# adityamwagh/SuperSLAM

Hardware: AMD Instinct MI355X
Metric: stereo pairs/sec (SPx2+LG) at 1376x376 (higher is better)
Workload: dtype f16; 1 GPU; configs[1]: SuperPoint x2 + select + gather + 1x LightGlue on 1376x376 stereo pairs; a step = 8 x 64 = 512 pairs per GPU resident in HBM (8 library calls of 64 pairs, different images per call), max_keypoints 600, seeded synthetic weights; pairs_per_call=64, max_keypoints=600, matches_last_call=1412, parallelism=replicated weights, pairs sharded over 1 rank(s), no data-path collective

## Files before the change

superslam_amd/csrc/api.hip:

```cpp
#include <algorithm>
#include <atomic>
#include <cmath>
#include <cstdarg>
#include <cstdlib>
#include <cstring>
#include <fstream>
#include <map>
#include <memory>
#include <mutex>
#include <string>
#include <vector>

#include "../../include/sship.h"
#include "../../include/superslam_hip/place_recognizer.hpp"
#include "kernels.h"

namespace sship {

static thread_local std::string g_err;
static void (*g_log_cb)(int, const char*) = nullptr;
static int g_profiling = 0;

void set_error(const std::string& msg) {
  g_err = msg;
// ... 492 lines not shown
  t.cand = cand.as<unsigned long long>(); t.cand_count = cnt.as<int>(); t.cap = cap; t.max_kp = max_kp;
  t.score_w = score_w;
  t.scale_x = static_cast<float>(input_w) / score_w;
  t.scale_y = static_cast<float>(input_h) / score_h;
  t.desc_h = desc_h; t.desc_w = desc_w; t.kp_xys = kp_xys; t.cell_h = cell_h; t.cell_w = cell_w; t.n_out = n_dev;
  t.n_cand_out = n_cand_dev;
  launch_topk(t, 1, s);
  SSHIP_HIP_CHECK(hipGetLastError());
  SSHIP_HIP_CHECK(hipStreamSynchronize(s));
  return SSHIP_OK;
}

struct sship_sp {
  sship_sp_config cfg{};
  hipStream_t stream = nullptr;
  float* w1a = nullptr;
  float* b1a = nullptr;
  _Float16* w1a_frag = nullptr;
  _Float16* w1a_fragb = nullptr;
  ConvW c1b, c2a, c2b, c3a, c3b, c4a, c4b, cPa, cPb, cDa, cDb;
  ConvW cDb32;
  sship_pool* pool = nullptr;
  int wsB = 0, wsH = 0, wsW = 0;
  DevBuf img, a1a, a1b, a2a, a2b, a3a, a3b, a4a, a4b, aPa, aDa, draw, logits, cand, cand_count;
  const void* cand_zero_ptr = nullptr; int cand_zero_n = 0;
  hipStream_t cand_zero_stream = nullptr;
  DevBuf kp, cell_h, cell_w, n_dev, desc_stage, gray_in;
  PinBuf h_kp, h_n, h_img;
  int cap = 0;
  float thr_f = 0.f;
  bool img_valid = false;
  struct Ring {
    int depth = 0, h = 0, w = 0, ch = 0;
    size_t img_bytes = 0;
    std::vector<void*> host, dev;
    std::vector<hipEvent_t> uploaded;
    hipStream_t copy_stream = nullptr;
    struct Pending { bool active = false; int slots[2] = {-1, -1}; int rc_pool = 0; hipEvent_t done = nullptr; void* h_kp = nullptr; void* h_n = nullptr; };
    std::vector<Pending> pending;
  } ring;
};

static void ring_free(sship_sp* sp);
static void sp_shapes(int H, int W, int& H2, int& W2, int& H4, int& W4, int& Hc, int& Wc) {
  H2 = H / 2; W2 = W / 2; H4 = H2 / 2; W4 = W2 / 2; Hc = H4 / 2; Wc = W4 / 2;
}

static int sp_ensure(sship_sp* sp, int B, int H, int W) {
  if (B <= sp->wsB && H == sp->wsH && W == sp->wsW) return SSHIP_OK;
  int H2, W2, H4, W4, Hc, Wc;
  sp_shapes(H, W, H2, W2, H4, W4, Hc, Wc);
  if (Hc < 1 || Wc < 1) return fail(SSHIP_ERR_INVALID, "image too small for SuperPoint (needs >= 8x8)");
  const size_t px1 = (size_t)B * H * W, px2 = (size_t)B * H2 * W2, px4 = (size_t)B * H4 * W4, pxc = (size_t)B * Hc * Wc;
  const int mk = sp->cfg.max_keypoints;
  SSHIP_HIP_CHECK(sp->img.ensure(px1));
  SSHIP_HIP_CHECK(sp->gray_in.ensure(px1 * 3));
  SSHIP_HIP_CHECK(sp->a1a.ensure(px1 * 64 * 2));
  SSHIP_HIP_CHECK(sp->a1b.ensure(px2 * 64 * 2));
  SSHIP_HIP_CHECK(sp->a2a.ensure(px2 * 64 * 2));
  SSHIP_HIP_CHECK(sp->a2b.ensure(px4 * 64 * 2));
  SSHIP_HIP_CHECK(sp->a3a.ensure(px4 * 128 * 2));
  SSHIP_HIP_CHECK(sp->a3b.ensure(pxc * 128 * 2));
  SSHIP_HIP_CHECK(sp->a4a.ensure(pxc * 128 * 2));
  SSHIP_HIP_CHECK(sp->a4b.ensure(pxc * 128 * 2));
  SSHIP_HIP_CHECK(sp->aPa.ensure(pxc * 256 * 2));
  SSHIP_HIP_CHECK(sp->aDa.ensure(pxc * 256 * 2));
  SSHIP_HIP_CHECK(sp->draw.ensure(pxc * 256 * 2));
  SSHIP_HIP_CHECK(sp->logits.ensure(pxc * kLogitStride * 4));
  sp->cap = Hc * 8 * Wc * 8;
  SSHIP_HIP_CHECK(sp->cand.ensure((size_t)B * sp->cap * 8));
  SSHIP_HIP_CHECK(sp->cand_count.ensure((size_t)B * 4));
  SSHIP_HIP_CHECK(sp->kp.ensure((size_t)B * mk * 3 * 4));
  SSHIP_HIP_CHECK(sp->cell_h.ensure((size_t)B * mk * 4));
  SSHIP_HIP_CHECK(sp->cell_w.ensure((size_t)B * mk * 4));
  SSHIP_HIP_CHECK(sp->n_dev.ensure((size_t)B * 4));
  SSHIP_HIP_CHECK(sp->h_kp.ensure((size_t)B * mk * 3 * 4));
  SSHIP_HIP_CHECK(sp->h_n.ensure((size_t)B * 4));
  SSHIP_HIP_CHECK(sp->h_img.ensure(px1 * 3));
  sp->wsB = B; sp->wsH = H; sp->wsW = W;
  return SSHIP_OK;
}

static int conv_mode() {
  static const int v = [] {
    const char* e = dev_env("SUPERSLAM_HIP_CONV");
    return (SSHIP_DEV_SWITCHES && e && std::string(e) == "strip") ? 2 : 1;
  }();
  return v;
}
static hipError_t conv3(const ConvW& w, const _Float16* in, _Float16* out, int B, int H, int W, bool pool, hipStream_t s) {
#if SSHIP_DEV_SWITCHES
  static const bool wino = [] { const char* e = dev_env("SUPERSLAM_HIP_CONV64"); return e && std::string(e) == "wino"; }();
  if (wino && w.w_wino && sp_conv3x3_wino_fits(H, W, w.cin, w.cout)) return sp_conv3x3_wino(w.w_wino, w.bias, in, out, B, H, W, pool, s);
  return conv_mode() == 1 ? sp_conv3x3_pp(w, in, out, B, H, W, pool, s) : sp_conv3x3_strip(w, in, out, B, H, W, pool, s);
#else
  return sp_conv3x3_pp(w, in, out, B, H, W, pool, s);
#endif
}
static bool conv2_fused(int B, int H2, int W2) {
#if SSHIP_DEV_SWITCHES
  static const std::string mode = [] { const char* e = dev_env("SUPERSLAM_HIP_CONV2"); return std::string(e ? e : ""); }();
  static const bool other = [] { const char* e = dev_env("SUPERSLAM_HIP_CONV64"); return e != nullptr; }();
  if (mode == "split" || other || conv_mode() != 1) return false;
#endif
  return sp_conv2ab_fused_fits(B, H2, W2, true);
}
static hipError_t conv3a_layer(const ConvW& w, const _Float16* in, _Float16* out, int B, int H, int W, hipStream_t s) {
#if SSHIP_DEV_SWITCHES
  static const bool roll = [] { const char* e = dev_env("SUPERSLAM_HIP_CONV3A"); return e && std::string(e) == "roll"; }();
  if (roll && conv_mode() == 1 && w.cin == 64 && w.cout == 128 && w.ct == 64 && sp_conv3a_roll_fits(B, H, W)) return sp_conv3a_roll(w, in, out, B, H, W, s);
#endif
  return conv3(w, in, out, B, H, W, false, s);
}
static hipError_t conv1ab(sship_sp* sp, const uint8_t* img, _Float16* out, int B, int H, int W, hipStream_t s);
static bool desc_dense_mode() {
  static const bool v = [] { const char* e = dev_env("SUPERSLAM_HIP_DESC"); return e && std::string(e) == "dense"; }();
  return v;
}
static hipError_t desc_head(sship_sp* sp, int img0, int Hc, int Wc, const int* cell_h, const int* cell_w, const int* n_dev, int B,
                            _Float16* out, size_t out_img_stride, hipStream_t s) {
  const int mk = sp->cfg.max_keypoints;
  if (desc_dense_mode()) {
    launch_desc_head_gather(sp->cDb32, sp->aDa.as<_Float16>() + (size_t)img0 * Hc * Wc * 256, Hc, Wc, cell_h, cell_w, n_dev, mk, B, out,
                            out_img_stride, s);
    return hipGetLastError();
  }
  return launch_desc_head_sparse(sp->cDa, sp->cDb32, sp->a4b.as<_Float16>() + (size_t)img0 * Hc * Wc * 128, Hc, Wc, cell_h, cell_w, n_dev,
                                 mk, B, out, out_img_stride, s);
}

static int sp_network(sship_sp* sp, const uint8_t* imgs, int B, int H, int W, hipStream_t s, bool dense_desc) {
  int H2, W2, H4, W4, Hc, Wc;
  sp_shapes(H, W, H2, W2, H4, W4, Hc, Wc);
  SSHIP_HIP_CHECK(conv1ab(sp, imgs, sp->a1b.as<_Float16>(), B, H, W, s));
  g_timer.mark_fine("sp_gpu_infer:encoder/conv1a+conv1b+pool", s);
  if (conv2_fused(B, H2, W2)) {
    SSHIP_HIP_CHECK(sp_conv2ab_fused(sp->c2a, sp->c2b, sp->a1b.as<_Float16>(), sp->a2b.as<_Float16>(), B, H2, W2, s));
    g_timer.mark_fine("sp_gpu_infer:encoder/conv2a+conv2b+pool", s);
  } else {
    SSHIP_HIP_CHECK(conv3(sp->c2a, sp->a1b.as<_Float16>(), sp->a2a.as<_Float16>(), B, H2, W2, false, s));
    g_timer.mark_fine("sp_gpu_infer:encoder/conv2a", s);
    SSHIP_HIP_CHECK(conv3(sp->c2b, sp->a2a.as<_Float16>(), sp->a2b.as<_Float16>(), B, H2, W2, true, s));
    g_timer.mark_fine("sp_gpu_infer:encoder/conv2b+pool", s);
  }
  SSHIP_HIP_CHECK(conv3a_layer(sp->c3a, sp->a2b.as<_Float16>(), sp->a3a.as<_Float16>(), B, H4, W4, s));
  g_timer.mark_fine("sp_gpu_infer:encoder/conv3a", s);
  SSHIP_HIP_CHECK(conv3(sp->c3b, sp->a3a.as<_Float16>(), sp->a3b.as<_Float16>(), B, H4, W4, true, s));
  g_timer.mark_fine("sp_gpu_infer:encoder/conv3b+pool", s);
  SSHIP_HIP_CHECK(conv3(sp->c4a, sp->a3b.as<_Float16>(), sp->a4a.as<_Float16>(), B, Hc, Wc, false, s));
  g_timer.mark_fine("sp_gpu_infer:encoder/conv4a", s);
  SSHIP_HIP_CHECK(conv3(sp->c4b, sp->a4a.as<_Float16>(), sp->a4b.as<_Float16>(), B, Hc, Wc, false, s));
  g_timer.mark(g_profiling >= 2 ? "sp_gpu_infer:encoder/conv4b" : "sp_gpu_infer:encoder", s);
  SSHIP_HIP_CHECK(conv3(sp->cPa, sp->a4b.as<_Float16>(), sp->aPa.as<_Float16>(), B, Hc, Wc, false, s));
  g_timer.mark_fine("sp_gpu_infer:heads/convPa", s);
  SSHIP_HIP_CHECK(sp_conv1x1_f32(sp->cPb, sp->aPa.as<_Float16>(), sp->logits.as<float>(), kLogitStride, B, Hc, Wc, s));
  if (dense_desc || desc_dense_mode()) SSHIP_HIP_CHECK(conv3(sp->cDa, sp->a4b.as<_Float16>(), sp->aDa.as<_Float16>(), B, Hc, Wc, false, s));
  if (dense_desc) SSHIP_HIP_CHECK(sp_conv1x1_f16(sp->cDb, sp->aDa.as<_Float16>(), sp->draw.as<_Float16>(), B, Hc, Wc, s));
  g_timer.mark(g_profiling >= 2 ? "sp_gpu_infer:heads/convPb" : "sp_gpu_infer:heads", s);
  return SSHIP_OK;
}

static int sp_select(sship_sp* sp, int B, int H, int W, float* scores_out, float* kp_out, int* n_out, hipStream_t s) {
  int H2, W2, H4, W4, Hc, Wc;
  sp_shapes(H, W, H2, W2, H4, W4, Hc, Wc);
  if (sp->cand_zero_ptr != sp->cand_count.p || sp->cand_zero_n < B || sp->cand_zero_stream != s)
    SSHIP_HIP_CHECK(hipMemsetAsync(sp->cand_count.p, 0, (size_t)B * 4, s));
  sp->cand_zero_ptr = sp->cand_count.p; sp->cand_zero_n = 0; sp->cand_zero_stream = s;
  NmsArgs a{};
  a.logits = sp->logits.as<float>(); a.ls = kLogitStride; a.B = B; a.H = Hc * 8; a.W = Wc * 8;
  a.radius = sp->cfg.nms_radius; a.thr_f = sp->thr_f; a.border = sp->cfg.remove_borders;
  a.cand = sp->cand.as<unsigned long long>(); a.cand_count = sp->cand_count.as<int>(); a.cap = sp->cap;
  a.scores_out = scores_out;
  launch_nms_tile(0, a, s);
  g_timer.mark_fine("sp_extract_stereo:select/nms_tile", s);
  TopkArgs t{};
  t.cand = a.cand; t.cand_count = a.cand_count; t.cap = sp->cap; t.max_kp = sp->cfg.max_keypoints;
  t.score_w = Wc * 8;
  t.scale_x = static_cast<float>(W) / (Wc * 8);
  t.scale_y = static_cast<float>(H) / (Hc * 8);
  t.desc_h = Hc; t.desc_w = Wc; t.kp_xys = kp_out; t.cell_h = sp->cell_h.as<int>(); t.cell_w = sp->cell_w.as<int>();
  t.n_out = n_out; t.n_cand_out = nullptr; t.reset_count = a.cand_count;
  launch_topk(t, B, s);
  SSHIP_HIP_CHECK(hipGetLastError());
  sp->cand_zero_n = B;
  g_timer.mark(g_profiling >= 2 ? "sp_extract_stereo:select/topk" : "sp_extract_stereo:select", s);
  return SSHIP_OK;
}

static hipError_t conv1ab(sship_sp* sp, const uint8_t* img, _Float16* out, int B, int H, int W, hipStream_t s) {
#if SSHIP_DEV_SWITCHES
  if (conv_mode() == 2) return sp_conv1ab_fused(sp->c1b, sp->w1a_frag, sp->b1a, img, out, B, H, W, s);
#endif
  return sp_conv1ab_pp(sp->c1b, sp->w1a_fragb, sp->b1a, img, out, B, H, W, s);
}

extern "C" int sship_sp_create(const sship_sp_config* cfg, sship_sp** out) {
  bind_thread();
  if (!cfg || !out || !cfg->weights_path) return fail(SSHIP_ERR_INVALID, "sp_create: null argument");
  if (cfg->max_keypoints <= 0 || cfg->max_keypoints > kMaxKp) return fail(SSHIP_ERR_INVALID, "sp_create: max_keypoints must be in [1, 4096]");
  if (cfg->nms_radius < 0 || cfg->nms_radius > 8) return fail(SSHIP_ERR_INVALID, "sp_create: nms_radius must be in [0, 8]");
  if (int rc = require_device()) return rc;
  StateDict sd; std::string err;
  if (!load_safetensors(cfg->weights_path, sd, err)) return fail(SSHIP_ERR_IO, err);
  std::unique_ptr<sship_sp, void (*)(sship_sp*)> sp(new sship_sp(), sship_sp_destroy);
// ... 69 lines not shown
  if (int rc = sship_pool_create(sp->cfg.pool_slots, sp->cfg.max_keypoints, SSHIP_DESC_DIM, &sp->pool)) return rc;
  *out = sp.release();
  return SSHIP_OK;
}
extern "C" void sship_sp_destroy(sship_sp* sp) {
  bind_thread();
  if (!sp) return;
  (void)hipDeviceSynchronize();
  for (ConvW* c : {&sp->c1b, &sp->c2a, &sp->c2b, &sp->c3a, &sp->c3b, &sp->c4a, &sp->c4b, &sp->cPa, &sp->cPb, &sp->cDa, &sp->cDb, &sp->cDb32})
    free_conv(*c);
  if (sp->w1a) (void)hipFree(sp->w1a);
  if (sp->b1a) (void)hipFree(sp->b1a);
  if (sp->w1a_frag) (void)hipFree(sp->w1a_frag);
  if (sp->w1a_fragb) (void)hipFree(sp->w1a_fragb);
  ring_free(sp);
  if (sp->pool) sship_pool_destroy(sp->pool);
  sp->pool = nullptr;
  if (sp->stream) (void)hipStreamDestroy(sp->stream);
  delete sp;
}
extern "C" int sship_sp_debug_activation(sship_sp* sp, int layer, void* out_host, unsigned long long bytes) {
  bind_thread();
  if (!sp || !out_host) return fail(SSHIP_ERR_INVALID, "sp_debug_activation: null argument");
  DevBuf* bufs[8] = {nullptr, &sp->a1b, &sp->a2a, &sp->a2b, &sp->a3a, &sp->a3b, &sp->a4a, &sp->a4b};
  if (layer < 1 || layer > 7 || !bufs[layer]->p || bytes > bufs[layer]->bytes) return fail(SSHIP_ERR_INVALID, "sp_debug_activation: bad layer / size");
  SSHIP_HIP_CHECK(hipDeviceSynchronize());
  SSHIP_HIP_CHECK(hipMemcpy(out_host, bufs[layer]->p, bytes, hipMemcpyDeviceToHost));
  return SSHIP_OK;
}
extern "C" sship_pool* sship_sp_pool(sship_sp* sp) {
  bind_thread(); return sp ? sp->pool : nullptr; }
extern "C" int sship_sp_max_keypoints(const sship_sp* sp) { return sp ? sp->cfg.max_keypoints : 0; }

extern "C" int sship_sp_extract_batch_device(sship_sp* sp, const uint8_t* imgs, int batch, int h, int w, void* desc_out,
                                             float* kp_out, int* n_out, void* stream) {
  bind_thread();
  if (!sp || !imgs || !desc_out || !kp_out || !n_out || batch <= 0) return fail(SSHIP_ERR_INVALID, "sp_extract_batch_device: bad arguments");
  hipStream_t s = static_cast<hipStream_t>(stream);
  if (int rc = sp_ensure(sp, batch, h, w)) return rc;
  if (g_profiling && imgs != sp->img.as<uint8_t>())
    SSHIP_HIP_CHECK(hipMemcpyAsync(sp->img.p, imgs, (size_t)batch * h * w, hipMemcpyDeviceToDevice, s));
  sp->img_valid = g_profiling != 0 || imgs == sp->img.as<uint8_t>();
  g_timer.begin(s);
  if (int rc = sp_network(sp, imgs, batch, h, w, s, false)) return rc;
  if (int rc = sp_select(sp, batch, h, w, nullptr, kp_out, n_out, s)) return rc;
  int H2, W2, H4, W4, Hc, Wc;
  sp_shapes(h, w, H2, W2, H4, W4, Hc, Wc);
  SSHIP_HIP_CHECK(desc_head(sp, 0, Hc, Wc, sp->cell_h.as<int>(), sp->cell_w.as<int>(), n_out, batch, static_cast<_Float16*>(desc_out),
                            (size_t)sp->cfg.max_keypoints * 256, s));
  g_timer.mark("sp_extract_stereo:gather", s);
  return SSHIP_OK;
}

extern "C" int sship_sp_dense(sship_sp* sp, const uint8_t* imgs, int batch, int h, int w, float* scores, void* desc_grid,
                              float* logits, void* stream) {
  bind_thread();
  if (!sp || !imgs || batch <= 0) return fail(SSHIP_ERR_INVALID, "sp_dense: bad arguments");
  hipStream_t s = static_cast<hipStream_t>(stream);
  if (int rc = sp_ensure(sp, batch, h, w)) return rc;
  if (int rc = sp_network(sp, imgs, batch, h, w, s, desc_grid != nullptr)) return rc;
  int H2, W2, H4, W4, Hc, Wc;
  sp_shapes(h, w, H2, W2, H4, W4, Hc, Wc);
  if (scores) {
    NmsArgs a{};
    a.logits = sp->logits.as<float>(); a.ls = kLogitStride; a.B = batch; a.H = Hc * 8; a.W = Wc * 8;
    a.radius = sp->cfg.nms_radius; a.scores_out = scores;
    launch_nms_tile(0, a, s);
  }
  if (desc_grid) launch_desc_dense_chw(sp->draw.as<_Float16>(), Hc * Wc, batch, static_cast<_Float16*>(desc_grid), s);
  if (logits) launch_logits_chw(sp->logits.as<float>(), kLogitStride, Hc * Wc, batch, logits, s);
  SSHIP_HIP_CHECK(hipGetLastError());
  return SSHIP_OK;
}

extern "C" int sship_mfma_probe(int random_operands, float* tflops) {
  bind_thread();
  if (!tflops) return fail(SSHIP_ERR_INVALID, "mfma_probe: null argument");
  if (int rc = require_device()) return rc;
  SSHIP_HIP_CHECK(mfma_probe(random_operands != 0, tflops));
  return SSHIP_OK;
}

extern "C" int sship_sp_bench_layer(sship_sp* sp, int layer, int batch, int h, int w, int iters, float* avg_ms,
                                    double* macs) {
  bind_thread();
  if (!sp || !avg_ms || iters <= 0 || layer < 0 || layer > 15) return fail(SSHIP_ERR_INVALID, "sp_bench_layer: bad arguments");
  if (batch > sp->wsB || h != sp->wsH || w != sp->wsW) return fail(SSHIP_ERR_INVALID, "sp_bench_layer: run the network at this shape first");
  if (layer <= 1 && !sp->img_valid)
    return fail(SSHIP_ERR_INVALID, "sp_bench_layer: the handle holds no copy of the last input - make one call with sship_set_profiling(1) first "
                                   "(a launch on stale / zero pixels runs at a higher clock than the real one)");
  int H2, W2, H4, W4, Hc, Wc;
  sp_shapes(h, w, H2, W2, H4, W4, Hc, Wc);
  hipStream_t s = sp->stream;
  _Float16 *a1a = sp->a1a.as<_Float16>(), *a1b = sp->a1b.as<_Float16>(), *a2a = sp->a2a.as<_Float16>(),
           *a2b = sp->a2b.as<_Float16>(), *a3a = sp->a3a.as<_Float16>(), *a3b = sp->a3b.as<_Float16>(),
           *a4a = sp->a4a.as<_Float16>(), *a4b = sp->a4b.as<_Float16>(), *aPa = sp->aPa.as<_Float16>(),
           *aDa = sp->aDa.as<_Float16>();
  auto run = [&]() -> hipError_t {
    switch (layer) {
      case 0: launch_conv1a(sp->img.as<uint8_t>(), sp->w1a, sp->b1a, a1a, batch, h, w, s); return hipGetLastError();
      case 1: return conv1ab(sp, sp->img.as<uint8_t>(), a1b, batch, h, w, s);
      case 15:
        if (!sp_conv2ab_fused_fits(batch, H2, W2, true)) return hipErrorInvalidValue;
        return sp_conv2ab_fused(sp->c2a, sp->c2b, a1b, a2b, batch, H2, W2, s);
      case 2: return conv3(sp->c2a, a1b, a2a, batch, H2, W2, false, s);
      case 3: return conv3(sp->c2b, a2a, a2b, batch, H2, W2, true, s);
      case 4: return conv3a_layer(sp->c3a, a2b, a3a, batch, H4, W4, s);
      case 5: return conv3(sp->c3b, a3a, a3b, batch, H4, W4, true, s);
      case 6: return conv3(sp->c4a, a3b, a4a, batch, Hc, Wc, false, s);
      case 7: return conv3(sp->c4b, a4a, a4b, batch, Hc, Wc, false, s);
      case 8: return conv3(sp->cPa, a4b, aPa, batch, Hc, Wc, false, s);
      case 9: return sp_conv1x1_f32(sp->cPb, aPa, sp->logits.as<float>(), kLogitStride, batch, Hc, Wc, s);
      case 10: return conv3(sp->cDa, a4b, aDa, batch, Hc, Wc, false, s);
      case 11: return sp_conv1x1_f16(sp->cDb, aDa, sp->draw.as<_Float16>(), batch, Hc, Wc, s);
      case 12: {
        if (hipError_t e = hipMemsetAsync(sp->cand_count.p, 0, (size_t)batch * 4, s)) return e;
        sp->cand_zero_n = 0;
        NmsArgs a{};
        a.logits = sp->logits.as<float>(); a.ls = kLogitStride; a.B = batch; a.H = Hc * 8; a.W = Wc * 8;
        a.radius = sp->cfg.nms_radius; a.thr_f = sp->thr_f; a.border = sp->cfg.remove_borders;
        a.cand = sp->cand.as<unsigned long long>(); a.cand_count = sp->cand_count.as<int>(); a.cap = sp->cap;
        launch_nms_tile(0, a, s);
        return hipGetLastError();
      }
      case 13: {
        TopkArgs t{};
        t.cand = sp->cand.as<unsigned long long>(); t.cand_count = sp->cand_count.as<int>(); t.cap = sp->cap;
        t.max_kp = sp->cfg.max_keypoints; t.score_w = Wc * 8;
        t.scale_x = static_cast<float>(w) / (Wc * 8); t.scale_y = static_cast<float>(h) / (Hc * 8);
        t.desc_h = Hc; t.desc_w = Wc; t.kp_xys = sp->kp.as<float>(); t.cell_h = sp->cell_h.as<int>(); t.cell_w = sp->cell_w.as<int>();
        t.n_out = sp->n_dev.as<int>(); t.n_cand_out = nullptr;
        launch_topk(t, batch, s);
        return hipGetLastError();
      }
      default:
        if (hipError_t e = sp->desc_stage.ensure((size_t)batch * sp->cfg.max_keypoints * 512)) return e;
        return desc_head(sp, 0, Hc, Wc, sp->cell_h.as<int>(), sp->cell_w.as<int>(), sp->n_dev.as<int>(), batch, sp->desc_stage.as<_Float16>(),
                         (size_t)sp->cfg.max_keypoints * 256, s);
    }
  };
  if (layer == 13 || layer == 14) {
    const int keep = layer;
    layer = 12; SSHIP_HIP_CHECK(run());
    layer = 13; SSHIP_HIP_CHECK(run());
    layer = keep;
  }
  const double px[12] = {(double)h * w, (double)h * w, (double)H2 * W2, (double)H2 * W2, (double)H4 * W4, (double)H4 * W4,
                         (double)Hc * Wc, (double)Hc * Wc, (double)Hc * Wc, (double)Hc * Wc, (double)Hc * Wc, (double)Hc * Wc};
  const double mpp[12] = {9.0 * 64, 576.0 * 64 + 9.0 * 64 , 576.0 * 64, 576.0 * 64, 576.0 * 128, 1152.0 * 128, 1152.0 * 128,
                          1152.0 * 128, 1152.0 * 256, 256.0 * 65, 1152.0 * 256, 256.0 * 256};
  if (macs) *macs = layer < 12 ? px[layer] * mpp[layer] * batch : layer == 15 ? (px[2] * mpp[2] + px[3] * mpp[3]) * batch : 0.0;
  SSHIP_HIP_CHECK(run());
  hipEvent_t e0, e1;
  SSHIP_HIP_CHECK(hipEventCreate(&e0));
  SSHIP_HIP_CHECK(hipEventCreate(&e1));
  SSHIP_HIP_CHECK(hipEventRecord(e0, s));
  for (int i = 0; i < iters; ++i) SSHIP_HIP_CHECK(run());
  SSHIP_HIP_CHECK(hipEventRecord(e1, s));
  SSHIP_HIP_CHECK(hipEventSynchronize(e1));
  float ms = 0.f;
  SSHIP_HIP_CHECK(hipEventElapsedTime(&ms, e0, e1));
  (void)hipEventDestroy(e0); (void)hipEventDestroy(e1);
  *avg_ms = ms / iters;
// ... 5 lines not shown
                           sship_features* const* outs) {
  if (channels != 1 && channels != 3) return fail(SSHIP_ERR_INVALID, "image must have 1 or 3 channels");
  if (h <= 0 || w <= 0 || stride < w * channels) return fail(SSHIP_ERR_INVALID, "bad image geometry");
  if (int rc = sp_ensure(sp, B, h, w)) return rc;
  hipStream_t s = sp->stream;
  const size_t row = (size_t)w * channels, img_bytes = row * h;
  uint8_t* hp = sp->h_img.as<uint8_t>();
  for (int b = 0; b < B; ++b)
    for (int y = 0; y < h; ++y) memcpy(hp + b * img_bytes + y * row, imgs[b] + (size_t)y * stride, row);
  if (channels == 1) {
    SSHIP_HIP_CHECK(hipMemcpyAsync(sp->img.p, hp, img_bytes * B, hipMemcpyHostToDevice, s));
  } else {
    SSHIP_HIP_CHECK(hipMemcpyAsync(sp->gray_in.p, hp, img_bytes * B, hipMemcpyHostToDevice, s));
    launch_bgr2gray(sp->gray_in.as<uint8_t>(), B * h * w, sp->img.as<uint8_t>(), s);
  }
  sp->img_valid = true;
  return sp_extract_device(sp, sp->img.as<uint8_t>(), B, h, w, outs);
}
static int sp_extract_enqueue(sship_sp* sp, const uint8_t* gray, int B, int h, int w, int* slots, int* rc_pool, float* h_kp, int* h_n) {
  hipStream_t s = sp->stream;
  g_timer.begin(s);
  *rc_pool = SSHIP_OK;
  for (int b = 0; b < B; ++b) slots[b] = -1;
  if (int rc = sp_network(sp, gray, B, h, w, s, false)) return rc;
  if (int rc = sp_select(sp, B, h, w, nullptr, sp->kp.as<float>(), sp->n_dev.as<int>(), s)) return rc;
  int H2, W2, H4, W4, Hc, Wc;
  sp_shapes(h, w, H2, W2, H4, W4, Hc, Wc);
  const int mk = sp->cfg.max_keypoints;
  auto give_back = [&](hipError_t e, const char* what) {
    (void)hipStreamSynchronize(s);
    for (int b = 0; b < B; ++b)
      if (slots[b] >= 0) { sship_pool_release(sp->pool, slots[b]); slots[b] = -1; }
    return fail(SSHIP_ERR_HIP, std::string(what) + ": " + hipGetErrorString(e));
  };
  for (int b = 0; b < B; ++b) {
    slots[b] = sship_pool_acquire(sp->pool);
    if (slots[b] < 0) { *rc_pool = SSHIP_ERR_POOL_EXHAUSTED; continue; }
    if (hipError_t e = desc_head(sp, b, Hc, Wc, sp->cell_h.as<int>() + (size_t)b * mk, sp->cell_w.as<int>() + (size_t)b * mk,
                                 sp->n_dev.as<int>() + b, 1, static_cast<_Float16*>(sship_pool_slot_ptr(sp->pool, slots[b])), 0, s))
      return give_back(e, "sp_extract: descriptor head");
  }
  g_timer.mark("sp_extract_stereo:gather", s);
  if (hipError_t e = hipMemcpyAsync(h_kp, sp->kp.p, (size_t)B * mk * 12, hipMemcpyDeviceToHost, s)) return give_back(e, "sp_extract: D2H keypoints");
  if (hipError_t e = hipMemcpyAsync(h_n, sp->n_dev.p, (size_t)B * 4, hipMemcpyDeviceToHost, s)) return give_back(e, "sp_extract: D2H counts");
  return SSHIP_OK;
}
static int sp_extract_finish(sship_sp* sp, int B, const int* slots, int rc_pool, const float* h_kp, const int* h_n, sship_features* const* outs) {
  const int mk = sp->cfg.max_keypoints;
  for (int b = 0; b < B; ++b) {
    const int n = h_n[b];
// ... 1027 lines not shown
```

superslam_amd/csrc/kernels.h:

```cpp
#pragma once
#include "common.h"

namespace sship {

constexpr int kMaxKp = 4096;
constexpr int kLogitStride = 68;

void launch_conv1a(const uint8_t* img, const float* w, const float* bias, _Float16* out, int B, int H, int W,
                   hipStream_t s);
struct NmsArgs {
  const float* logits;
  int ls;
  const float* scores_in;
  int B, H, W;
  int radius;
  float thr_f;
  int border;
  unsigned long long* cand;
  int* cand_count;
  int cap;
  float* scores_out;
  float* scores_raw_out;
};
float threshold_as_float(double thr);
void launch_nms_tile(int loader, const NmsArgs& a, hipStream_t s);

struct TopkArgs {
  const unsigned long long* cand;
  const int* cand_count;
  int* reset_count;
  int cap, max_kp;
  int score_w;
  float scale_x, scale_y;
  int desc_h, desc_w;
  float* kp_xys;
  int* cell_h;
  int* cell_w;
  int* n_out;
  int* n_cand_out;
};
void launch_topk(const TopkArgs& a, int B, hipStream_t s);
void launch_threshold_scan(const float* scores, int H, int W, float thr_f, int border, unsigned long long* cand,
                           int* cand_count, int cap, hipStream_t s);
void launch_gather_hwc(bool raw, const _Float16* grid, int C, int gh, int gw, size_t img_stride, const int* cell_h,
                       const int* cell_w, const int* n_dev, int n_host, int max_kp, int B, _Float16* out,
                       hipStream_t s);
void launch_gather_chw(const _Float16* grid, int C, int gh, int gw, const int* cell_h, const int* cell_w, int n,
// ... 90 lines not shown
```

superslam_amd/csrc/sp_kernels.hip:

```cpp
#include "kernels.h"

namespace sship {

__global__ __launch_bounds__(256) void k_conv1a(const uint8_t* __restrict__ img, const float* __restrict__ w,
                                                const float* __restrict__ bias, _Float16* __restrict__ out,
                                                int B, int H, int W) {
  __shared__ float s_w[9 * 64];
  for (int i = threadIdx.x; i < 576; i += 256) s_w[i] = w[i];
  __syncthreads();
  const int grp = threadIdx.x & 7;
  const int q = blockIdx.x * 32 + (threadIdx.x >> 3);
  const int qw = (W + 3) >> 2;
  if (q >= B * H * qw) return;
  const int xq = q % qw, y = (q / qw) % H, b = q / (qw * H);
  const int x0 = xq * 4;
  float in[3][6];
#pragma unroll
  for (int dy = 0; dy < 3; ++dy)
#pragma unroll
    for (int dx = 0; dx < 6; ++dx) {
      const int yy = y + dy - 1, xx = x0 + dx - 1;
      float v = 0.f;
      if (yy >= 0 && yy < H && xx >= 0 && xx < W) {
        v = (float)(_Float16)((float)img[((size_t)b * H + yy) * W + xx] * (1.0f / 255.0f));
// ... 31 lines not shown
                   hipStream_t s) {
  const int quads = B * H * ((W + 3) / 4);
  hipLaunchKernelGGL(k_conv1a, dim3((quads + 31) / 32), dim3(256), 0, s, img, w, bias, out, B, H, W);
}

constexpr int NT_H = 32, NT_W = 64, NHALO = 8, NLH = NT_H + 2 * NHALO, NLW = NT_W + 2 * NHALO, NLS = NLW + 4;
constexpr int NMS_SLOTS = NT_H * NT_W / 256;

__device__ __forceinline__ float max3(float a, float b, float c) { return fmaxf(fmaxf(a, b), c); }

__device__ __forceinline__ void window9x4(const float (&v)[12], float (&o)[4]) {
  const float c = fmaxf(max3(v[3], v[4], v[5]), max3(v[6], v[7], v[8]));
  o[0] = fmaxf(c, max3(v[0], v[1], v[2]));
  o[1] = fmaxf(c, max3(v[1], v[2], v[9]));
  o[2] = fmaxf(c, max3(v[2], v[9], v[10]));
  o[3] = fmaxf(c, max3(v[9], v[10], v[11]));
}

constexpr int NMS_PEND = 256;
#ifndef SSHIP_NMS_XCD
#define SSHIP_NMS_XCD 1
#endif

template <int LOADER, int RT>
__global__ __launch_bounds__(256) void k_nms_tile(NmsArgs a) {
  __shared__ __attribute__((aligned(16))) float s_buf[NLH * NLS + NLH * NT_W];
  __shared__ unsigned long long s_pend[NMS_PEND];
  __shared__ int s_cnt, s_base;
  float* s_s = s_buf;
  float* s_r = s_buf + NLH * NLS;
  unsigned long long* s_c = reinterpret_cast<unsigned long long*>(s_buf);
  static_assert(sizeof(s_buf) >= NT_H * NT_W * 8, "candidate list must fit the aliased buffers");
  const int tiles_x = (a.W + NT_W - 1) / NT_W, tiles_y = (a.H + NT_H - 1) / NT_H;
  const int ntiles = a.B * tiles_x * tiles_y;
  const int tid = threadIdx.x, lane = tid & 63;
  constexpr int NCELL = (NLH / 8) * (NLW / 8);
  const int cell = tid >> 2, qd = tid & 3;
  const int cyl = cell / (NLW / 8), cxl = cell % (NLW / 8);
  float4 pv[4];
  float pd = 0.f;
  bool pin = false;
  auto fetch = [&](int tt) {
    if constexpr (LOADER == 0) {
      const int Hc = a.H >> 3, Wc = a.W >> 3;
      int q = tt;
      const int ftx = q % tiles_x; q /= tiles_x;
      const int fty = q % tiles_y;
      const int fb = q / tiles_y;
      const int cy = ((fty * NT_H - NHALO) >> 3) + cyl, cx = ((ftx * NT_W - NHALO) >> 3) + cxl;
      pin = tid < NCELL * 4 && cy >= 0 && cy < Hc && cx >= 0 && cx < Wc;
      const int ccy = min(max(cy, 0), Hc - 1), ccx = min(max(cx, 0), Wc - 1);
      const float* lp = a.logits + ((size_t)(fb * Hc + ccy) * Wc + ccx) * a.ls;
#pragma unroll
      for (int i = 0; i < 4; ++i) pv[i] = *reinterpret_cast<const float4*>(lp + qd * 16 + i * 4);
      pd = lp[64];
    }
  };
  int pend_n = 0, pend_b = 0;
  int ticket = 0;
  auto flush_pending = [&]() {
    if (pend_n) {
      const int base = s_base;
      for (int i = tid; i < pend_n; i += 256)
        if (base + i < a.cap) a.cand[(size_t)pend_b * a.cap + base + i] = s_pend[i];
    }
  };
  const bool xcd_map = SSHIP_NMS_XCD && (gridDim.x & 7) == 0 && gridDim.x >= 8;
  const int xq = xcd_map ? (int)(blockIdx.x >> 3) : (int)blockIdx.x, xQ = xcd_map ? (int)(gridDim.x >> 3) : (int)gridDim.x;
  const int per = xcd_map ? (ntiles + 7) >> 3 : ntiles, xbase = xcd_map ? (int)(blockIdx.x & 7) * per : 0;
  const int t_end = min(per, ntiles - xbase);
  if (xq < t_end) fetch(xbase + xq);
#pragma unroll 1
  for (int tl = xq; tl < t_end; tl += xQ) {
    const int tile = xbase + tl;
    int t = tile;
    const int tx = t % tiles_x; t /= tiles_x;
    const int ty = t % tiles_y;
    const int b = t / tiles_y;
    const int x0 = tx * NT_W - NHALO, y0 = ty * NT_H - NHALO;
    if (tid == 0) {
      s_cnt = 0;
      if (pend_n) s_base = ticket;
    }
    if constexpr (LOADER == 0) {
      if (tid < NCELL * 4) {
        float v[16];
        const bool in = pin;
        const float d = in ? pd : 0.f;
#pragma unroll
        for (int i = 0; i < 4; ++i) {
          v[4 * i] = in ? pv[i].x : 0.f; v[4 * i + 1] = in ? pv[i].y : 0.f;
          v[4 * i + 2] = in ? pv[i].z : 0.f; v[4 * i + 3] = in ? pv[i].w : 0.f;
        }
        float m = d;
#pragma unroll
        for (int i = 0; i < 16; ++i) m = fmaxf(m, v[i]);
        m = fmaxf(m, __shfl_xor(m, 1, 64));
        m = fmaxf(m, __shfl_xor(m, 2, 64));
        float sum = 0.f;
#pragma unroll
        for (int i = 0; i < 16; ++i) { v[i] = __expf(v[i] - m); sum += v[i]; }
        sum += __shfl_xor(sum, 1, 64);
        sum += __shfl_xor(sum, 2, 64);
        sum += __expf(d - m);
        const float inv = 1.0f / sum;
#pragma unroll
        for (int r = 0; r < 2; ++r) {
          float* dst = s_s + (cyl * 8 + qd * 2 + r) * NLS + cxl * 8;
#pragma unroll
          for (int h = 0; h < 2; ++h) {
            float4 o;
            o.x = in ? v[r * 8 + h * 4 + 0] * inv : -INFINITY;
            o.y = in ? v[r * 8 + h * 4 + 1] * inv : -INFINITY;
            o.z = in ? v[r * 8 + h * 4 + 2] * inv : -INFINITY;
            o.w = in ? v[r * 8 + h * 4 + 3] * inv : -INFINITY;
            *reinterpret_cast<float4*>(dst + h * 4) = o;
          }
        }
      }
      if (tl + xQ < t_end) fetch(tile + xQ);
    } else {
      for (int i = tid; i < NLH * NLW; i += 256) {
        const int ly = i / NLW, lx = i % NLW;
        const int gy = y0 + ly, gx = x0 + lx;
        float sc = -INFINITY;
        if (gy >= 0 && gy < a.H && gx >= 0 && gx < a.W) sc = a.scores_in[((size_t)b * a.H + gy) * a.W + gx];
        s_s[ly * NLS + lx] = sc;
      }
    }
    __syncthreads();
    flush_pending();
    if constexpr (RT == 4) {
      for (int it = tid; it < NLH * (NT_W / 4); it += 256) {
        const int row = it >> 4, seg = it & 15;
        const float* p = s_s + row * NLS + NHALO - 4 + 4 * seg;
        float v[12], o[4];
#pragma unroll
        for (int q = 0; q < 3; ++q) {
          const float4 t4 = *reinterpret_cast<const float4*>(p + 4 * q);
          v[4 * q] = t4.x; v[4 * q + 1] = t4.y; v[4 * q + 2] = t4.z; v[4 * q + 3] = t4.w;
        }
        window9x4(v, o);
        *reinterpret_cast<float4*>(s_r + row * NT_W + 4 * seg) = make_float4(o[0], o[1], o[2], o[3]);
// ... 76 lines not shown
          if (base + i < a.cap) a.cand[(size_t)b * a.cap + base + i] = s_c[i];
      } else if (n > 0) {
        if (tid < n) s_pend[tid] = s_c[tid];
        if (tid == 0) ticket = atomicAdd(&a.cand_count[b], n);
        pend_n = n; pend_b = b;
      }
    }
    __syncthreads();
  }
  if (pend_n) {
    if (tid == 0) s_base = ticket;
    __syncthreads();
    flush_pending();
  }
}

float threshold_as_float(double thr) {
  float f = (float)thr;
  while ((double)f > thr) f = nextafterf(f, -INFINITY);
  while (!((double)f > thr)) f = nextafterf(f, INFINITY);
  return f;
}

void launch_nms_tile(int loader, const NmsArgs& a, hipStream_t s) {
  const int ntiles = a.B * ((a.W + NT_W - 1) / NT_W) * ((a.H + NT_H - 1) / NT_H);
  const int tiles = ntiles < 5 * cu_count() ? ntiles : 5 * cu_count();
  const bool r4 = a.radius == 4;
  if (loader == 0) {
    if (r4) hipLaunchKernelGGL((k_nms_tile<0, 4>), dim3(tiles), dim3(256), 0, s, a);
    else hipLaunchKernelGGL((k_nms_tile<0, -1>), dim3(tiles), dim3(256), 0, s, a);
  } else {
    if (r4) hipLaunchKernelGGL((k_nms_tile<1, 4>), dim3(tiles), dim3(256), 0, s, a);
    else hipLaunchKernelGGL((k_nms_tile<1, -1>), dim3(tiles), dim3(256), 0, s, a);
  }
}



constexpr int TOPK_CACHE = 8;

__global__ __launch_bounds__(1024) void k_topk(TopkArgs a) {
  __shared__ unsigned long long s_key[kMaxKp];
  __shared__ int s_hist[256];
  __shared__ unsigned long long s_prefix;
  __shared__ int s_remaining, s_cnt, s_done;
  __shared__ unsigned long long s_out[1024];
  const int b = blockIdx.x, tid = threadIdx.x, lane = tid & 63;
  const int n_cand = a.cand_count[b];
  const int M = min(n_cand, a.cap);
  const int K = min(M, a.max_kp);
// ... 291 lines not shown
```

Measured before the change: 5488 pairs/s.

## Fuse convPb 1x1 head into NMS tile kernel via MFMA loader

Adds a third NMS loader that computes the 65-channel convPb logits per tile directly from the convPa activations with MFMA, holding the weights in registers and LDS. The separate 1x1 conv launch and the fp32 logit map it wrote to and read back from HBM go away. The a2a and logits buffers are now allocated lazily, only on paths that need them. In exchange the NMS kernel does more work per tile, runs fewer workgroups (2 per CU) and has higher register pressure.

Measured after the change: 5471 pairs/s, median of 2. No clear change (-0.3%).

```diff
diff --git a/superslam_amd/csrc/api.hip b/superslam_amd/csrc/api.hip
--- a/superslam_amd/csrc/api.hip
+++ b/superslam_amd/csrc/api.hip
@@ -538,7 +538,8 @@
   ConvW cDb32;
   sship_pool* pool = nullptr;
   int wsB = 0, wsH = 0, wsW = 0;
-  DevBuf img, a1a, a1b, a2a, a2b, a3a, a3b, a4a, a4b, aPa, aDa, draw, logits, cand, cand_count;
+  DevBuf img, a1a, a1b, a2a, a2b, a3a, a3b, a4a, a4b, aPa, aDa, draw, logits, cand, cand_count, n_cand;
+  int a2a_images = 0, logits_images = 0;
   const void* cand_zero_ptr = nullptr; int cand_zero_n = 0;
   hipStream_t cand_zero_stream = nullptr;
   DevBuf kp, cell_h, cell_w, n_dev, desc_stage, gray_in;
@@ -573,7 +574,6 @@
   SSHIP_HIP_CHECK(sp->gray_in.ensure(px1 * 3));
   SSHIP_HIP_CHECK(sp->a1a.ensure(px1 * 64 * 2));
   SSHIP_HIP_CHECK(sp->a1b.ensure(px2 * 64 * 2));
-  SSHIP_HIP_CHECK(sp->a2a.ensure(px2 * 64 * 2));
   SSHIP_HIP_CHECK(sp->a2b.ensure(px4 * 64 * 2));
   SSHIP_HIP_CHECK(sp->a3a.ensure(px4 * 128 * 2));
   SSHIP_HIP_CHECK(sp->a3b.ensure(pxc * 128 * 2));
@@ -582,10 +582,10 @@
   SSHIP_HIP_CHECK(sp->aPa.ensure(pxc * 256 * 2));
   SSHIP_HIP_CHECK(sp->aDa.ensure(pxc * 256 * 2));
   SSHIP_HIP_CHECK(sp->draw.ensure(pxc * 256 * 2));
-  SSHIP_HIP_CHECK(sp->logits.ensure(pxc * kLogitStride * 4));
   sp->cap = Hc * 8 * Wc * 8;
   SSHIP_HIP_CHECK(sp->cand.ensure((size_t)B * sp->cap * 8));
   SSHIP_HIP_CHECK(sp->cand_count.ensure((size_t)B * 4));
+  SSHIP_HIP_CHECK(sp->n_cand.ensure((size_t)B * 4));
   SSHIP_HIP_CHECK(sp->kp.ensure((size_t)B * mk * 3 * 4));
   SSHIP_HIP_CHECK(sp->cell_h.ensure((size_t)B * mk * 4));
   SSHIP_HIP_CHECK(sp->cell_w.ensure((size_t)B * mk * 4));
@@ -594,7 +594,14 @@
   SSHIP_HIP_CHECK(sp->h_n.ensure((size_t)B * 4));
   SSHIP_HIP_CHECK(sp->h_img.ensure(px1 * 3));
   sp->wsB = B; sp->wsH = H; sp->wsW = W;
-  return SSHIP_OK;
+  sp->a2a_images = 0; sp->logits_images = 0;
+  return SSHIP_OK;
+}
+static hipError_t sp_lazy_a2a(sship_sp* sp) { return sp->a2a.ensure((size_t)sp->wsB * (sp->wsH / 2) * (sp->wsW / 2) * 64 * 2); }
+static hipError_t sp_lazy_logits(sship_sp* sp) {
+  int H2, W2, H4, W4, Hc, Wc;
+  sp_shapes(sp->wsH, sp->wsW, H2, W2, H4, W4, Hc, Wc);
+  return sp->logits.ensure((size_t)sp->wsB * Hc * Wc * kLogitStride * 4);
 }
 
 static int conv_mode() {
@@ -628,6 +635,13 @@
 #endif
   return conv3(w, in, out, B, H, W, false, s);
 }
+static bool tail_fused(const sship_sp* sp, int B, int Hc, int Wc) {
+#if SSHIP_DEV_SWITCHES
+  if (const char* e = dev_env("SUPERSLAM_HIP_TAIL"))
+    if (std::string(e) == "split") return false;
+#endif
+  return sp->cfg.nms_radius == 4 && sp->cPb.w_q && sp->cPb.cin == 256 && sp->cPb.cout == 65 && nms_tile_fused_fits(B, Hc * 8, Wc * 8);
+}
 static hipError_t conv1ab(sship_sp* sp, const uint8_t* img, _Float16* out, int B, int H, int W, hipStream_t s);
 static bool desc_dense_mode() {
   static const bool v = [] { const char* e = dev_env("SUPERSLAM_HIP_DESC"); return e && std::string(e) == "dense"; }();
@@ -645,16 +659,19 @@
                                  mk, B, out, out_img_stride, s);
 }
 
-static int sp_network(sship_sp* sp, const uint8_t* imgs, int B, int H, int W, hipStream_t s, bool dense_desc) {
+static int sp_network(sship_sp* sp, const uint8_t* imgs, int B, int H, int W, hipStream_t s, bool dense_desc, bool want_logits) {
   int H2, W2, H4, W4, Hc, Wc;
   sp_shapes(H, W, H2, W2, H4, W4, Hc, Wc);
+  sp->a2a_images = 0; sp->logits_images = 0;
   SSHIP_HIP_CHECK(conv1ab(sp, imgs, sp->a1b.as<_Float16>(), B, H, W, s));
   g_timer.mark_fine("sp_gpu_infer:encoder/conv1a+conv1b+pool", s);
   if (conv2_fused(B, H2, W2)) {
     SSHIP_HIP_CHECK(sp_conv2ab_fused(sp->c2a, sp->c2b, sp->a1b.as<_Float16>(), sp->a2b.as<_Float16>(), B, H2, W2, s));
     g_timer.mark_fine("sp_gpu_infer:encoder/conv2a+conv2b+pool", s);
   } else {
+    SSHIP_HIP_CHECK(sp_lazy_a2a(sp));
     SSHIP_HIP_CHECK(conv3(sp->c2a, sp->a1b.as<_Float16>(), sp->a2a.as<_Float16>(), B, H2, W2, false, s));
+    sp->a2a_images = B;
     g_timer.mark_fine("sp_gpu_infer:encoder/conv2a", s);
     SSHIP_HIP_CHECK(conv3(sp->c2b, sp->a2a.as<_Float16>(), sp->a2b.as<_Float16>(), B, H2, W2, true, s));
     g_timer.mark_fine("sp_gpu_infer:encoder/conv2b+pool", s);
@@ -669,10 +686,16 @@
   g_timer.mark(g_profiling >= 2 ? "sp_gpu_infer:encoder/conv4b" : "sp_gpu_infer:encoder", s);
   SSHIP_HIP_CHECK(conv3(sp->cPa, sp->a4b.as<_Float16>(), sp->aPa.as<_Float16>(), B, Hc, Wc, false, s));
   g_timer.mark_fine("sp_gpu_infer:heads/convPa", s);
-  SSHIP_HIP_CHECK(sp_conv1x1_f32(sp->cPb, sp->aPa.as<_Float16>(), sp->logits.as<float>(), kLogitStride, B, Hc, Wc, s));
+  if (want_logits) {
+    SSHIP_HIP_CHECK(sp_lazy_logits(sp));
+    SSHIP_HIP_CHECK(sp_conv1x1_f32(sp->cPb, sp->aPa.as<_Float16>(), sp->logits.as<float>(), kLogitStride, B, Hc, Wc, s));
+    sp->logits_images = B;
+  }
   if (dense_desc || desc_dense_mode()) SSHIP_HIP_CHECK(conv3(sp->cDa, sp->a4b.as<_Float16>(), sp->aDa.as<_Float16>(), B, Hc, Wc, false, s));
   if (dense_desc) SSHIP_HIP_CHECK(sp_conv1x1_f16(sp->cDb, sp->aDa.as<_Float16>(), sp->draw.as<_Float16>(), B, Hc, Wc, s));
-  g_timer.mark(g_profiling >= 2 ? "sp_gpu_infer:heads/convPb" : "sp_gpu_infer:heads", s);
+  if (g_profiling < 2) g_timer.mark("sp_gpu_infer:heads", s);
+  else if (want_logits) g_timer.mark("sp_gpu_infer:heads/convPb", s);
+  else if (dense_desc || desc_dense_mode()) g_timer.mark("sp_gpu_infer:heads/convDa", s);
   return SSHIP_OK;
 }
 
@@ -683,11 +706,18 @@
     SSHIP_HIP_CHECK(hipMemsetAsync(sp->cand_count.p, 0, (size_t)B * 4, s));
   sp->cand_zero_ptr = sp->cand_count.p; sp->cand_zero_n = 0; sp->cand_zero_stream = s;
   NmsArgs a{};
-  a.logits = sp->logits.as<float>(); a.ls = kLogitStride; a.B = B; a.H = Hc * 8; a.W = Wc * 8;
+  a.ls = kLogitStride; a.B = B; a.H = Hc * 8; a.W = Wc * 8;
   a.radius = sp->cfg.nms_radius; a.thr_f = sp->thr_f; a.border = sp->cfg.remove_borders;
   a.cand = sp->cand.as<unsigned long long>(); a.cand_count = sp->cand_count.as<int>(); a.cap = sp->cap;
   a.scores_out = scores_out;
-  launch_nms_tile(0, a, s);
+  if (sp->logits_images >= B) {
+    a.logits = sp->logits.as<float>();
+    launch_nms_tile(0, a, s);
+  } else {
+    if (!tail_fused(sp, B, Hc, Wc)) return fail(SSHIP_ERR_INVALID, "sp_select: the network call left no logit map");
+    a.act = sp->aPa.as<_Float16>(); a.wpb = sp->cPb.w_q; a.bpb = sp->cPb.bias;
+    launch_nms_tile(2, a, s);
+  }
   g_timer.mark_fine("sp_extract_stereo:select/nms_tile", s);
   TopkArgs t{};
   t.cand = a.cand; t.cand_count = a.cand_count; t.cap = sp->cap; t.max_kp = sp->cfg.max_keypoints;
@@ -695,7 +725,7 @@
   t.scale_x = static_cast<float>(W) / (Wc * 8);
   t.scale_y = static_cast<float>(H) / (Hc * 8);
   t.desc_h = Hc; t.desc_w = Wc; t.kp_xys = kp_out; t.cell_h = sp->cell_h.as<int>(); t.cell_w = sp->cell_w.as<int>();
-  t.n_out = n_out; t.n_cand_out = nullptr; t.reset_count = a.cand_count;
+  t.n_out = n_out; t.n_cand_out = sp->n_cand.as<int>(); t.reset_count = a.cand_count;
   launch_topk(t, B, s);
   SSHIP_HIP_CHECK(hipGetLastError());
   sp->cand_zero_n = B;
@@ -811,8 +841,10 @@
 extern "C" int sship_sp_debug_activation(sship_sp* sp, int layer, void* out_host, unsigned long long bytes) {
   bind_thread();
   if (!sp || !out_host) return fail(SSHIP_ERR_INVALID, "sp_debug_activation: null argument");
-  DevBuf* bufs[8] = {nullptr, &sp->a1b, &sp->a2a, &sp->a2b, &sp->a3a, &sp->a3b, &sp->a4a, &sp->a4b};
-  if (layer < 1 || layer > 7 || !bufs[layer]->p || bytes > bufs[layer]->bytes) return fail(SSHIP_ERR_INVALID, "sp_debug_activation: bad layer / size");
+  DevBuf* bufs[12] = {nullptr, &sp->a1b, &sp->a2a, &sp->a2b, &sp->a3a, &sp->a3b, &sp->a4a, &sp->a4b, &sp->n_cand, &sp->cand, &sp->cell_h, &sp->cell_w};
+  if (layer < 1 || layer > 11 || !bufs[layer]->p || bytes > bufs[layer]->bytes) return fail(SSHIP_ERR_INVALID, "sp_debug_activation: bad layer / size");
+  if (layer == 2 && !sp->a2a_images)
+    return fail(SSHIP_ERR_INVALID, "sp_debug_activation: the last call ran conv2a + conv2b as one launch and wrote no conv2a map");
   SSHIP_HIP_CHECK(hipDeviceSynchronize());
   SSHIP_HIP_CHECK(hipMemcpy(out_host, bufs[layer]->p, bytes, hipMemcpyDeviceToHost));
   return SSHIP_OK;
@@ -831,10 +863,10 @@
     SSHIP_HIP_CHECK(hipMemcpyAsync(sp->img.p, imgs, (size_t)batch * h * w, hipMemcpyDeviceToDevice, s));
   sp->img_valid = g_profiling != 0 || imgs == sp->img.as<uint8_t>();
   g_timer.begin(s);
-  if (int rc = sp_network(sp, imgs, batch, h, w, s, false)) return rc;
-  if (int rc = sp_select(sp, batch, h, w, nullptr, kp_out, n_out, s)) return rc;
   int H2, W2, H4, W4, Hc, Wc;
   sp_shapes(h, w, H2, W2, H4, W4, Hc, Wc);
+  if (int rc = sp_network(sp, imgs, batch, h, w, s, false, !tail_fused(sp, batch, Hc, Wc))) return rc;
+  if (int rc = sp_select(sp, batch, h, w, nullptr, kp_out, n_out, s)) return rc;
   SSHIP_HIP_CHECK(desc_head(sp, 0, Hc, Wc, sp->cell_h.as<int>(), sp->cell_w.as<int>(), n_out, batch, static_cast<_Float16*>(desc_out),
                             (size_t)sp->cfg.max_keypoints * 256, s));
   g_timer.mark("sp_extract_stereo:gather", s);
@@ -847,7 +879,7 @@
   if (!sp || !imgs || batch <= 0) return fail(SSHIP_ERR_INVALID, "sp_dense: bad arguments");
   hipStream_t s = static_cast<hipStream_t>(stream);
   if (int rc = sp_ensure(sp, batch, h, w)) return rc;
-  if (int rc = sp_network(sp, imgs, batch, h, w, s, desc_grid != nullptr)) return rc;
+  if (int rc = sp_network(sp, imgs, batch, h, w, s, desc_grid != nullptr, true)) return rc;
   int H2, W2, H4, W4, Hc, Wc;
   sp_shapes(h, w, H2, W2, H4, W4, Hc, Wc);
   if (scores) {
@@ -881,6 +913,9 @@
   int H2, W2, H4, W4, Hc, Wc;
   sp_shapes(h, w, H2, W2, H4, W4, Hc, Wc);
   hipStream_t s = sp->stream;
+  const bool uses_a2a = layer == 2 || layer == 3, uses_logits = layer == 9 || (layer >= 12 && layer <= 14);
+  if (uses_a2a) SSHIP_HIP_CHECK(sp_lazy_a2a(sp));
+  if (uses_logits) SSHIP_HIP_CHECK(sp_lazy_logits(sp));
   _Float16 *a1a = sp->a1a.as<_Float16>(), *a1b = sp->a1b.as<_Float16>(), *a2a = sp->a2a.as<_Float16>(),
            *a2b = sp->a2b.as<_Float16>(), *a3a = sp->a3a.as<_Float16>(), *a3b = sp->a3b.as<_Float16>(),
            *a4a = sp->a4a.as<_Float16>(), *a4b = sp->a4b.as<_Float16>(), *aPa = sp->aPa.as<_Float16>(),
@@ -918,7 +953,7 @@
         t.max_kp = sp->cfg.max_keypoints; t.score_w = Wc * 8;
         t.scale_x = static_cast<float>(w) / (Wc * 8); t.scale_y = static_cast<float>(h) / (Hc * 8);
         t.desc_h = Hc; t.desc_w = Wc; t.kp_xys = sp->kp.as<float>(); t.cell_h = sp->cell_h.as<int>(); t.cell_w = sp->cell_w.as<int>();
-        t.n_out = sp->n_dev.as<int>(); t.n_cand_out = nullptr;
+        t.n_out = sp->n_dev.as<int>(); t.n_cand_out = sp->n_cand.as<int>();
         launch_topk(t, batch, s);
         return hipGetLastError();
       }
@@ -928,6 +963,18 @@
                          (size_t)sp->cfg.max_keypoints * 256, s);
     }
   };
+  if (uses_a2a && sp->a2a_images < batch) {
+    const int keep = layer;
+    layer = 2; SSHIP_HIP_CHECK(run());
+    layer = keep;
+    sp->a2a_images = batch;
+  }
+  if (uses_logits && sp->logits_images < batch) {
+    const int keep = layer;
+    layer = 9; SSHIP_HIP_CHECK(run());
+    layer = keep;
+    sp->logits_images = batch;
+  }
   if (layer == 13 || layer == 14) {
     const int keep = layer;
     layer = 12; SSHIP_HIP_CHECK(run());
@@ -979,10 +1026,10 @@
   g_timer.begin(s);
   *rc_pool = SSHIP_OK;
   for (int b = 0; b < B; ++b) slots[b] = -1;
-  if (int rc = sp_network(sp, gray, B, h, w, s, false)) return rc;
-  if (int rc = sp_select(sp, B, h, w, nullptr, sp->kp.as<float>(), sp->n_dev.as<int>(), s)) return rc;
   int H2, W2, H4, W4, Hc, Wc;
   sp_shapes(h, w, H2, W2, H4, W4, Hc, Wc);
+  if (int rc = sp_network(sp, gray, B, h, w, s, false, !tail_fused(sp, B, Hc, Wc))) return rc;
+  if (int rc = sp_select(sp, B, h, w, nullptr, sp->kp.as<float>(), sp->n_dev.as<int>(), s)) return rc;
   const int mk = sp->cfg.max_keypoints;
   auto give_back = [&](hipError_t e, const char* what) {
     (void)hipStreamSynchronize(s);
diff --git a/superslam_amd/csrc/kernels.h b/superslam_amd/csrc/kernels.h
--- a/superslam_amd/csrc/kernels.h
+++ b/superslam_amd/csrc/kernels.h
@@ -21,8 +21,12 @@
   int cap;
   float* scores_out;
   float* scores_raw_out;
+  const _Float16* act;
+  const _Float16* wpb;
+  const float* bpb;
 };
 float threshold_as_float(double thr);
+bool nms_tile_fused_fits(int B, int H, int W);
 void launch_nms_tile(int loader, const NmsArgs& a, hipStream_t s);
 
 struct TopkArgs {
diff --git a/superslam_amd/csrc/sp_kernels.hip b/superslam_amd/csrc/sp_kernels.hip
--- a/superslam_amd/csrc/sp_kernels.hip
+++ b/superslam_amd/csrc/sp_kernels.hip
@@ -77,13 +77,23 @@
 #define SSHIP_NMS_XCD 1
 #endif
 
-template <int LOADER, int RT>
-__global__ __launch_bounds__(256) void k_nms_tile(NmsArgs a) {
-  __shared__ __attribute__((aligned(16))) float s_buf[NLH * NLS + NLH * NT_W];
+constexpr int NLG_LD = 68, NLG_CELLS = 64;
+
+template <int LOADER, int RT, int MREG = 4>
+__global__ __launch_bounds__(256, LOADER == 2 ? (MREG == 4 ? 2 : 3) : 1) void k_nms_tile(NmsArgs a) {
+  constexpr bool FUSED = LOADER == 2;
+  static_assert(!FUSED || RT == 4, "the convPa loader exists for the production radius only");
+  constexpr int WR = FUSED ? MREG : 1, WL = FUSED ? 4 - MREG : 0;
+  constexpr int NSR = FUSED && NLG_CELLS * NLG_LD > NLH * NT_W ? NLG_CELLS * NLG_LD : NLH * NT_W;
+  __shared__ __attribute__((aligned(16))) float s_buf[NLH * NLS + NSR];
   __shared__ unsigned long long s_pend[NMS_PEND];
   __shared__ int s_cnt, s_base;
+  __shared__ __attribute__((aligned(16))) _Float16 s_wl[WL ? WL * 8 * 512 : 8];
+  __shared__ __attribute__((aligned(16))) _Float16 s_a4[FUSED ? 8 * 4 * 8 : 8];
+  __shared__ __attribute__((aligned(16))) float s_pb[FUSED ? 80 : 4];
   float* s_s = s_buf;
   float* s_r = s_buf + NLH * NLS;
+  float* s_lg = s_r;
   unsigned long long* s_c = reinterpret_cast<unsigned long long*>(s_buf);
   static_assert(sizeof(s_buf) >= NT_H * NT_W * 8, "candidate list must fit the aliased buffers");
   const int tiles_x = (a.W + NT_W - 1) / NT_W, tiles_y = (a.H + NT_H - 1) / NT_H;
@@ -95,7 +105,35 @@
   float4 pv[4];
   float pd = 0.f;
   bool pin = false;
+  const int wv = tid >> 6, fn = lane & 15, fkb = lane >> 4, fcell = wv * 16 + fn;
+  h8_t wr[WR][8];
+  h8_t pf[8];
+  if constexpr (FUSED) {
+    if (tid < 32) *reinterpret_cast<uint4*>(s_a4 + tid * 8) = *reinterpret_cast<const uint4*>(a.wpb + (size_t)64 * 256 + (tid >> 2) * 32 + (tid & 3) * 8);
+    if (tid < 80) s_pb[tid] = tid < 65 ? a.bpb[tid] : 0.f;
+    for (int u = tid; u < WL * 8 * 64; u += 256) {
+      const int m = WR + (u >> 9), ks = (u >> 6) & 7, l = u & 63;
+      *reinterpret_cast<uint4*>(s_wl + u * 8) = *reinterpret_cast<const uint4*>(a.wpb + (size_t)(16 * m + (l & 15)) * 256 + ks * 32 + (l >> 4) * 8);
+    }
+#pragma unroll
+    for (int m = 0; m < WR; ++m)
+#pragma unroll
+      for (int ks = 0; ks < 8; ++ks) wr[m][ks] = *reinterpret_cast<const h8_t*>(a.wpb + (size_t)(16 * m + fn) * 256 + ks * 32 + fkb * 8);
+    __syncthreads();
+  }
   auto fetch = [&](int tt) {
+    if constexpr (FUSED) {
+      const int Hc = a.H >> 3, Wc = a.W >> 3;
+      int q = tt;
+      const int ftx = q % tiles_x; q /= tiles_x;
+      const int fty = q % tiles_y;
+      const int fb = q / tiles_y;
+      const int cy = fty * (NT_H / 8) - 1 + fcell / (NLW / 8), cx = ftx * (NT_W / 8) - 1 + fcell % (NLW / 8);
+      const int ccy = min(max(cy, 0), Hc - 1), ccx = min(max(cx, 0), Wc - 1);
+      const _Float16* p = a.act + ((size_t)(fb * Hc + ccy) * Wc + ccx) * 256 + fkb * 8;
+#pragma unroll
+      for (int ks = 0; ks < 8; ++ks) pf[ks] = *reinterpret_cast<const h8_t*>(p + ks * 32);
+    }
     if constexpr (LOADER == 0) {
       const int Hc = a.H >> 3, Wc = a.W >> 3;
       int q = tt;
@@ -137,7 +175,41 @@
       s_cnt = 0;
       if (pend_n) s_base = ticket;
     }
-    if constexpr (LOADER == 0) {
+    if constexpr (FUSED) {
+      f4x_t acc[5];
+#pragma unroll
+      for (int m = 0; m < 5; ++m) acc[m] = *reinterpret_cast<const f4x_t*>(s_pb + 16 * m + 4 * fkb);
+#pragma unroll
+      for (int ks = 0; ks < 8; ++ks) {
+        h8_t a4 = *reinterpret_cast<const h8_t*>(s_a4 + (ks * 4 + fkb) * 8);
+        if (fn != 0) a4 = h8_t{0, 0, 0, 0, 0, 0, 0, 0};
+#pragma unroll
+        for (int m = 0; m < 4; ++m) {
+          if (m < WR)
+            acc[m] = __builtin_amdgcn_mfma_f32_16x16x32_f16(wr[m < WR ? m : 0][ks], pf[ks], acc[m], 0, 0, 0);
+          else
+            acc[m] = __builtin_amdgcn_mfma_f32_16x16x32_f16(*reinterpret_cast<const h8_t*>(s_wl + (((m - WR) * 8 + ks) * 64 + lane) * 8), pf[ks],
+                                                            acc[m], 0, 0, 0);
+        }
+        acc[4] = __builtin_amdgcn_mfma_f32_16x16x32_f16(a4, pf[ks], acc[4], 0, 0, 0);
+      }
+      float* o = s_lg + fcell * NLG_LD + 4 * fkb;
+#pragma unroll
+      for (int m = 0; m < 4; ++m) *reinterpret_cast<f4x_t*>(o + 16 * m) = acc[m];
+      if (fkb == 0) o[64] = acc[4][0];
+      if (tl + xQ < t_end) fetch(tile + xQ);
+      __syncthreads();
+      if (tid < NCELL * 4) {
+        const int Hc = a.H >> 3, Wc = a.W >> 3;
+        const int cy = (y0 >> 3) + cyl, cx = (x0 >> 3) + cxl;
+        pin = cy >= 0 && cy < Hc && cx >= 0 && cx < Wc;
+        const float* lp = s_lg + cell * NLG_LD;
+#pragma unroll
+        for (int i = 0; i < 4; ++i) pv[i] = *reinterpret_cast<const float4*>(lp + qd * 16 + i * 4);
+        pd = lp[64];
+      }
+    }
+    if constexpr (LOADER == 0 || FUSED) {
       if (tid < NCELL * 4) {
         float v[16];
         const bool in = pin;
@@ -173,7 +245,8 @@
           }
         }
       }
-      if (tl + xQ < t_end) fetch(tile + xQ);
+      if constexpr (LOADER == 0)
+        if (tl + xQ < t_end) fetch(tile + xQ);
     } else {
       for (int i = tid; i < NLH * NLW; i += 256) {
         const int ly = i / NLW, lx = i % NLW;
@@ -296,10 +369,19 @@
   return f;
 }
 
+bool nms_tile_fused_fits(int B, int H, int W) {
+  return B > 0 && H >= 8 && W >= 8 && (H & 7) == 0 && (W & 7) == 0 && (long long)B * (H >> 3) * (W >> 3) < (1ll << 31);
+}
+
 void launch_nms_tile(int loader, const NmsArgs& a, hipStream_t s) {
   const int ntiles = a.B * ((a.W + NT_W - 1) / NT_W) * ((a.H + NT_H - 1) / NT_H);
   const int tiles = ntiles < 5 * cu_count() ? ntiles : 5 * cu_count();
   const bool r4 = a.radius == 4;
+  if (loader == 2) {
+    const int wgs = ntiles < 2 * cu_count() ? ntiles : 2 * cu_count();
+    hipLaunchKernelGGL((k_nms_tile<2, 4>), dim3(wgs), dim3(256), 0, s, a);
+    return;
+  }
   if (loader == 0) {
     if (r4) hipLaunchKernelGGL((k_nms_tile<0, 4>), dim3(tiles), dim3(256), 0, s, a);
     else hipLaunchKernelGGL((k_nms_tile<0, -1>), dim3(tiles), dim3(256), 0, s, a);
```
